# g1257/LanczosPlusPlus

Measured on AMD Instinct MI355X. Metric: Lanczos iterations/sec + SpMV achieved HBM GB/s vs roofline, 1/2/4/8 GPU, higher is better.
Workload: dtype f64

## Files before the change

lanczosplusplus_amd/csrc/lpp_pb_kernels.h:

```cpp
#pragma once
#include "lpp_kernels.h"
#include "lpp_pb_geom.h"

namespace lpp {

struct PbUpArgs {
	const uint32_t* tw;
	const int32_t* tw_off;
	const uint16_t* tw_len;
	int G;
	double gval[kPbMaxGroups];
	const double* dict;
	const uint8_t* dcode;
	int64_t n_up, pitch, n_blk;
	int spb;
	const double* y;
	double* u;
	double* partial;
	EpiScale sc;
	double* wbuf;
	double* ybuf;
	const double* g_a;
	const double* g_b2;
};

constexpr int kPbPreMax = 6;
constexpr int kPbPreMin = 1;
template <int GT> struct PbWords {
	uint2 w[GT][kPbPreMax];
	int nc[GT];
	double yo;
};

__device__ __forceinline__ uint32_t pb_lo8(uint32_t w)
{
	uint32_t r;
	asm("v_lshlrev_b32_sdwa %0, %1, %2 dst_sel:DWORD dst_unused:UNUSED_PAD src0_sel:DWORD src1_sel:WORD_0" : "=v"(r) : "v"(3u), "v"(w));
	return r;
}
__device__ __forceinline__ uint32_t pb_hi8(uint32_t w)
{
	uint32_t r;
	asm("v_lshlrev_b32_sdwa %0, %1, %2 dst_sel:DWORD dst_unused:UNUSED_PAD src0_sel:DWORD src1_sel:WORD_1" : "=v"(r) : "v"(3u), "v"(w));
	return r;
}
typedef __attribute__((address_space(3))) const double pb_lds_cdouble;
__device__ __forceinline__ double pb_lds_abs(uint32_t byte_addr) { return *(pb_lds_cdouble*)(uintptr_t)byte_addr; }

__device__ __forceinline__ void pb_lds_barrier()
{
	asm volatile("s_waitcnt lgkmcnt(0)" ::: "memory");
	__builtin_amdgcn_s_barrier();
}

template <bool DOT, int GT, bool CHAIN = false, int PRE0 = kPbPre> __global__ __launch_bounds__(kPbUpThreads, 4) void k_pb_up(PbUpArgs a)
{
	extern __shared__ __attribute__((aligned(16))) unsigned char lds_raw[];
	double* win = (double*)lds_raw;
	uint8_t* dcode_s = (uint8_t*)(win + a.pitch + kPbZeroSlots);
	int32_t* off_s = (int32_t*)(lds_raw + pb_up_meta_offset(a.pitch));
	uint16_t* len_s = (uint16_t*)(off_s + a.spb * a.G);
	double* dict_s = (double*)(lds_raw + pb_up_dict_offset(a.pitch, a.spb, a.G));
	double* smem = dict_s + 256;
	for (int i = threadIdx.x; i < 256; i += kPbUpThreads) dict_s[i] = a.dict[i];
	for (int i = threadIdx.x; i < a.spb * a.G; i += kPbUpThreads) {
		off_s[i] = a.tw_off[i];
		len_s[i] = a.tw_len[i];
	}
	double alpha, beta;
	epi_coeffs(a.sc, alpha, beta);
	double gco = 0.0;
	if (CHAIN && a.g_a) {
		gco = *a.g_a;
		const double b2 = *a.g_b2;
		if (sqrt(b2) >= 1e-10) gco /= b2;
	}
	constexpr int NW = kPbUpThreads / 64;
	constexpr int GG = GT > 0 ? GT : 1;
	const int lane = threadIdx.x & 63, wave = __builtin_amdgcn_readfirstlane((int)(threadIdx.x >> 6));
	const int p2 = (int)(a.pitch >> 1), p16 = (int)(a.pitch >> 4);
	double dot = 0.0;
	const uint2* const tw2 = (const uint2*)a.tw;
	const uint4* const tw4 = (const uint4*)a.tw;
	double* const uout = a.u;
	const int spb = a.spb, n_up = (int)a.n_up, G = a.G;
	double gv[GG];
#pragma unroll
	for (int g = 0; g < GG; g++) gv[g] = a.gval[g];
	auto gather4 = [=](const uint2& w, double& s0, double& s1) __attribute__((always_inline)) {
		s0 += pb_lds_abs(pb_lo8(w.x));
		s1 += pb_lds_abs(pb_hi8(w.x));
		s0 += pb_lds_abs(pb_lo8(w.y));
		s1 += pb_lds_abs(pb_hi8(w.y));
	};
	for (int64_t blk = blockIdx.x; blk < a.n_blk; blk += gridDim.x) {
		const double2* yb = (const double2*)(a.y + blk * a.pitch);
		const uint4* db = (const uint4*)(a.dcode + blk * a.pitch);
		const int64_t rowbase = blk * a.pitch;
		pb_lds_barrier();
		if (CHAIN) {
			double2* const wb = (double2*)(a.wbuf + rowbase);
			const double2* const yo = (const double2*)(a.ybuf + rowbase);
			const int di = min((int)threadIdx.x, p16 - 1);
			const uint4 dc0 = db[di];
			constexpr int NS = 4;
			for (int i0 = threadIdx.x; i0 < p2; i0 += NS * kPbUpThreads) {
				double2 wv[NS], yv[NS];
				int idx[NS];
#pragma unroll
				for (int q = 0; q < NS; q++) idx[q] = min(i0 + q * kPbUpThreads, p2 - 1);
#pragma unroll
				for (int q = 0; q < NS; q++) wv[q] = wb[idx[q]];
				if (gco != 0.0) {
#pragma unroll
					for (int q = 0; q < NS; q++) yv[q] = yo[idx[q]];
#pragma unroll
					for (int q = 0; q < NS; q++) {
						wv[q].x -= gco * yv[q].x;
						wv[q].y -= gco * yv[q].y;
						if (i0 + q * kPbUpThreads < p2) wb[idx[q]] = wv[q];
					}
				}
#pragma unroll
				for (int q = 0; q < NS; q++)
					if (i0 + q * kPbUpThreads < p2) ((double2*)win)[idx[q]] = wv[q];
			}
			((uint4*)dcode_s)[di] = dc0;
			for (int i0 = threadIdx.x + kPbUpThreads; i0 < p16; i0 += kPbUpThreads) ((uint4*)dcode_s)[i0] = db[i0];
		} else {
			constexpr int NS = 8;
			for (int pass = 0; pass < 8 / NS; pass++) {
				double2 t[NS];
				int idx[NS];
#pragma unroll
				for (int q = 0; q < NS; q++) idx[q] = min((int)threadIdx.x + (pass * NS + q) * kPbUpThreads, p2 - 1);
#pragma unroll
				for (int q = 0; q < NS; q++) t[q] = yb[idx[q]];
#pragma unroll
				for (int q = 0; q < NS; q++) ((double2*)win)[idx[q]] = t[q];
			}
			const int di = min((int)threadIdx.x, p16 - 1);
			((uint4*)dcode_s)[di] = db[di];
			for (int i0 = threadIdx.x + 8 * kPbUpThreads; i0 < p2; i0 += kPbUpThreads) ((double2*)win)[i0] = yb[i0];
			for (int i0 = threadIdx.x + kPbUpThreads; i0 < p16; i0 += kPbUpThreads) ((uint4*)dcode_s)[i0] = db[i0];
		}
		if (threadIdx.x < kPbZeroSlots) win[a.pitch + threadIdx.x] = 0.0;
		pb_lds_barrier();
		const double* const yold = CHAIN ? a.ybuf + rowbase : nullptr;
		auto own = [=](int j, double& yc, double& dv) __attribute__((always_inline)) {
			const int iu = min(j * 64 + lane, n_up - 1);
			yc = win[iu];
			dv = dict_s[dcode_s[iu]];
		};
		auto finish = [=, &dot](int j, double acc, double yc, double dv, double yo) __attribute__((always_inline)) {
			const int iu = j * 64 + lane;
			acc = fma(dv, yc, acc);
			if (iu < n_up) {
				const double uv = CHAIN ? fma(beta, yo, alpha * acc) : alpha * acc;
				__builtin_nontemporal_store(uv, &uout[rowbase + iu]);
				if (DOT) dot += yc * uv;
			}
		};
		auto epilogue = [=](int j, double acc, double yo = 0.0) __attribute__((always_inline)) {
			double yc, dv;
			own(j, yc, dv);
			finish(j, acc, yc, dv, yo);
		};
		if (GT > 0) {
			auto load_words = [=](int j, PbWords<GG>& s) __attribute__((always_inline)) {
#pragma unroll
				for (int g = 0; g < GG; g++) {
					s.nc[g] = __builtin_amdgcn_readfirstlane((int)len_s[j * GG + g]);
					constexpr int PRE0_ = PRE0;
					const int depth = pb_depth(GG, g, PRE0_);
					if (kPbPairs) {
						const uint4* wp4 = tw4 + (size_t)__builtin_amdgcn_readfirstlane(off_s[j * GG + g]) * 64 + lane;
#pragma unroll
						for (int c = 0; c < kPbPreMax; c += 2)
							if (c < depth) {
								const uint4 t = wp4[(c >> 1) * 64];
								s.w[g][c] = uint2 { t.x, t.y };
								s.w[g][c + 1] = uint2 { t.z, t.w };
							}
					} else {
						const uint2* wp = tw2 + (size_t)off_s[j * GG + g] * 64 + lane;
#pragma unroll
						for (int c = 0; c < kPbPreMax; c++)
							if (c < depth && (c < kPbPreMin || c < s.nc[g])) s.w[g][c] = wp[c * 64];
					}
				}
				if (CHAIN) s.yo = yold[min(j * 64 + lane, n_up - 1)];
			};
			auto group_sum = [=](int j, int g, int nc, const uint2* w, int depth) __attribute__((always_inline)) {
				double s0 = 0.0, s1 = 0.0;
				constexpr int BT = 2;
#pragma unroll
				for (int c = 0; c < kPbPreMax; c += BT) {
					if (c >= depth) continue;
					if (BT >= 3 && c + 3 <= depth && nc >= c + 3) {
						gather4(w[c], s0, s1);
						gather4(w[c + 1], s0, s1);
						gather4(w[c + 2], s0, s1);
					} else if (c + 2 <= depth && nc >= c + 2) {
						gather4(w[c], s0, s1);
						gather4(w[c + 1], s0, s1);
					} else if (nc >= c + 1) {
						gather4(w[c], s0, s1);
					}
				}
				if (nc > depth) {
					if (kPbPairs) {
						const uint4* wp4 = tw4 + (size_t)off_s[j * GG + g] * 64 + lane;
						for (int c = depth; c < nc; c += 2) {
							const uint4 t = wp4[(c >> 1) * 64];
							gather4(uint2 { t.x, t.y }, s0, s1);
							if (c + 1 < nc) gather4(uint2 { t.z, t.w }, s0, s1);
						}
					} else {
						const uint2* wp = tw2 + (size_t)off_s[j * GG + g] * 64 + lane;
						for (int c = depth; c < nc; c++) {
							const uint2 wr = wp[c * 64];
							gather4(wr, s0, s1);
						}
					}
				}
				return s0 + s1;
			};
			auto compute = [=](int j, const PbWords<GG>& s) __attribute__((always_inline)) {
				double yc, dv;
				own(j, yc, dv);
				double acc = 0.0;
#pragma unroll
				for (int g = 0; g < GG; g++) acc = fma(gv[g], group_sum(j, g, s.nc[g], s.w[g], pb_depth(GG, g, PRE0)), acc);
				if (kPbPairs) {
#pragma unroll
					for (int g = 0; g < GG; g++)
#pragma unroll
						for (int c = 0; c < kPbPreMax; c += 2)
							if (c < pb_depth(GG, g, PRE0)) asm volatile("" ::"v"(s.w[g][c].x));
				}
				if (CHAIN) asm volatile("" ::"v"(s.yo));
				finish(j, acc, yc, dv, CHAIN ? s.yo : 0.0);
			};
			PbWords<GG> wa, wb;
			int j = wave;
			if (j < spb) {
				load_words(j, wa);
				for (; j + 2 * NW < spb; j += 2 * NW) {
					load_words(j + NW, wb);
					compute(j, wa);
					load_words(j + 2 * NW, wa);
					compute(j + NW, wb);
				}
				if (j + NW < spb) {
					load_words(j + NW, wb);
					compute(j, wa);
					compute(j + NW, wb);
				} else {
					compute(j, wa);
				}
			}
		} else {
			for (int j = wave; j < spb; j += NW) {
				double acc = 0.0;
				const double yo_g = CHAIN ? yold[min(j * 64 + lane, n_up - 1)] : 0.0;
				uint2 wn[4];
				int ncn = __builtin_amdgcn_readfirstlane((int)len_s[j * G]);
				auto load4 = [=](size_t off, int c0, int nc, uint2* w) __attribute__((always_inline)) {
					if (kPbPairs) {
						const uint4* wp4 = tw4 + off * 64 + lane;
#pragma unroll
						for (int q = 0; q < 4; q += 2) {
							const uint4 t = wp4[((c0 + q) >> 1) * 64];
							w[q] = uint2 { t.x, t.y };
							w[q + 1] = uint2 { t.z, t.w };
						}
					} else {
						const uint2* wp = tw2 + off * 64 + lane;
#pragma unroll
						for (int q = 0; q < 4; q++)
							if (c0 + q < nc) w[q] = wp[(c0 + q) * 64];
					}
				};
				size_t offn = (size_t)__builtin_amdgcn_readfirstlane(off_s[j * G]);
				load4(offn, 0, ncn, wn);
				for (int g = 0; g < G; g++) {
					const int nc = ncn;
					const size_t off = offn;
					uint2 w[4];
#pragma unroll
					for (int q = 0; q < 4; q++) w[q] = wn[q];
					if (g + 1 < G) {
						ncn = __builtin_amdgcn_readfirstlane((int)len_s[j * G + g + 1]);
						offn = (size_t)__builtin_amdgcn_readfirstlane(off_s[j * G + g + 1]);
						load4(offn, 0, ncn, wn);
					}
					double s0 = 0.0, s1 = 0.0;
#pragma unroll
					for (int q = 0; q < 4; q++)
						if (q < nc) gather4(w[q], s0, s1);
					for (int c0 = 4; c0 < nc; c0 += 4) {
						uint2 wr[4];
						load4(off, c0, nc, wr);
#pragma unroll
						for (int q = 0; q < 4; q++)
							if (c0 + q < nc) gather4(wr[q], s0, s1);
						if (kPbPairs) asm volatile("" ::"v"(wr[0].x), "v"(wr[2].x));
					}
					acc = fma(a.gval[g], s0 + s1, acc);
				}
				epilogue(j, acc, yo_g);
			}
		}
	}
	if (DOT) {
		const double r = block_sum_n<kPbUpThreads / 64>(dot, smem);
		if (threadIdx.x == 0) a.partial[blockIdx.x] = r;
	}
}

template <int CTRL> __device__ __forceinline__ double dpp_shr(double v)
{
	const long long b = __double_as_longlong(v);
	const int lo = __builtin_amdgcn_update_dpp(0, (int)b, CTRL, 0xf, 0xf, true);
	const int hi = __builtin_amdgcn_update_dpp(0, (int)(b >> 32), CTRL, 0xf, 0xf, true);
	return __longlong_as_double((long long)(((unsigned long long)(unsigned)hi << 32) | (unsigned)lo));
}
__device__ __forceinline__ double wave_sum_rows(double v)
{
	v += dpp_shr<0x111>(v);
	v += dpp_shr<0x112>(v);
	v += dpp_shr<0x114>(v);
	v += dpp_shr<0x118>(v);
	auto lane_val = [&](int l) __attribute__((always_inline)) {
		const long long b = __double_as_longlong(v);
		const int lo = __builtin_amdgcn_readlane((int)b, l), hi = __builtin_amdgcn_readlane((int)(b >> 32), l);
		return __longlong_as_double((long long)(((unsigned long long)(unsigned)hi << 32) | (unsigned)lo));
	};
	return ((lane_val(15) + lane_val(31)) + lane_val(47)) + lane_val(63);
}

__device__ inline void pb_down_fill_image(uint32_t* row, int32_t* len, uint32_t* place, int stride, int rowcap, const int32_t* order, const int64_t* c_ptr,
                                          const int32_t* c_col, const uint8_t* c_code, int64_t b0, int nown, uint32_t rowmul, int tid, int nthreads)
{
	constexpr int BPT = 8;
	for (int il = tid; il < nown; il += nthreads) {
		const int64_t b = order[b0 + il];
		row[il] = (uint32_t)b * rowmul;
		len[il] = (int32_t)(c_ptr[b + 1] - c_ptr[b]);
	}
	for (int i = tid; i < nown * rowcap; i += nthreads) {
		const int il = i / rowcap, k = i - il * rowcap;
		const int64_t b = order[b0 + il];
		const int64_t p0 = c_ptr[b];
		const bool in = k < (int)(c_ptr[b + 1] - p0);
		const int64_t bl = order[b0 + (il & ~(BPT - 1))];
		const int64_t pl = c_ptr[bl];
		const int32_t fill = k < (int)(c_ptr[bl + 1] - pl) ? c_col[pl + k] : (int32_t)bl;
		place[il * stride + k] = ((uint32_t)(in ? c_col[p0 + k] : fill) & 0xffffffu) | ((uint32_t)(in ? c_code[p0 + k] : (uint8_t)0) << 24);
	}
}

struct PbDownArgs {
	int64_t pitch, n_blk;
	int npanels;
	int ids_per_wg;
	int rounds, ids_per_round;
	const uint4* image;
	int rowcap;
	const int64_t* c_ptr;
	const int32_t* c_col;
	const uint8_t* c_code;
	const int32_t* order;
	const double* dict;
	const double* y;
	double* z;
	const double* u_in;
	const double* shift;
	double* partial;
	EpiScale sc;
	int* pace;
	int u_has_beta;
	const double2* cdict;
	int pf_lead;
};

template <int THREADS, bool RMW = false, bool WIDE = false, bool CPLX = false, bool PF = false> __global__ __launch_bounds__(THREADS) void k_pb_down(PbDownArgs a)
{
	extern __shared__ __attribute__((aligned(16))) unsigned char lds_raw[];
	__shared__ double dict_s[CPLX ? 512 : 256];
	const int stride = pb_down_stride(a.rowcap);
	uint32_t* row_s = (uint32_t*)lds_raw;
	int32_t* len_s = (int32_t*)(row_s + a.ids_per_round);
	uint32_t* place_s = (uint32_t*)(lds_raw + (((size_t)a.ids_per_round * 8 + 15) & ~(size_t)15));
	__shared__ double smem_d[THREADS / 64];
	__shared__ int task_s[3];
	if (PF && threadIdx.x < 3) task_s[threadIdx.x] = 0;
	for (int i = threadIdx.x; i < (CPLX ? 512 : 256); i += THREADS) dict_s[i] = CPLX ? ((const double*)a.cdict)[i] : a.dict[i];
	double alpha, beta;
	epi_coeffs(a.sc, alpha, beta);
	double dot = 0.0, nrm = 0.0;
	const double sh = RMW ? *a.shift : 0.0;
	constexpr int LPL = 8;
	constexpr int BPT = 64 / LPL;
	constexpr int LSH = 7;
	const int lane = threadIdx.x & 63, wave = threadIdx.x >> 6, sub = lane / LPL, c = lane & (LPL - 1);
	const int nx = (gridDim.x & 7) == 0 ? 8 : 1;
	const int grp = nx == 8 ? (int)(blockIdx.x & 7) : 0;
	const int slot = nx == 8 ? (int)(blockIdx.x >> 3) : (int)blockIdx.x;
	const int nslots = (int)(gridDim.x / nx);
	const uint32_t rowbytes = WIDE ? (uint32_t)((a.pitch * 8) >> LSH) : (uint32_t)(a.pitch * 8);
	const int64_t b0w = (int64_t)slot * a.ids_per_wg;
	const int nown_w = (int)max((int64_t)0, min((int64_t)a.ids_per_wg, a.n_blk - b0w));
	const int rounds = a.rounds;
	const int tcap = (a.ids_per_round + BPT - 1) / BPT;
	double* const tsum_s = (double*)(lds_raw + pb_down_lds_bytes(a.ids_per_round, a.rowcap));
	auto fold = [&](int q, int ng) __attribute__((always_inline)) {
		if (wave != 0) return;
		const double* const t = tsum_s + (size_t)(q & 1) * 2 * tcap;
		double sd = 0.0, sn = 0.0;
		for (int i = lane; i < ng; i += 64) {
			sd += t[i];
			if (RMW) sn += t[tcap + i];
		}
		sd = wave_sum(sd);
		if (RMW) sn = wave_sum(sn);
		if (lane == 0) {
			dot += sd;
			nrm += sn;
		}
	};
	int64_t b0 = b0w;
	int nown = rounds == 1 ? nown_w : 0;
	auto build_image = [&](int r) __attribute__((always_inline)) {
		b0 = b0w + (int64_t)r * a.ids_per_round;
		nown = rounds == 1 ? nown_w : max(0, min(a.ids_per_round, nown_w - r * a.ids_per_round));
		if (rounds > 1 && a.image) {
			const int n4 = (int)(pb_down_lds_bytes(a.ids_per_round, a.rowcap) >> 4);
			const uint4* const src = a.image + ((size_t)slot * rounds + r) * (size_t)n4;
			for (int i = threadIdx.x; i < n4; i += THREADS) {
				uint4 v = src[i];
				if (4 * i < a.ids_per_round) {
					v.x *= rowbytes;
					v.y *= rowbytes;
					v.z *= rowbytes;
					v.w *= rowbytes;
				}
				((uint4*)lds_raw)[i] = v;
			}
			return;
		}
		pb_down_fill_image(row_s, len_s, place_s, stride, a.rowcap, a.order, a.c_ptr, a.c_col, a.c_code, b0, nown, rowbytes, (int)threadIdx.x, THREADS);
	};
	if (rounds == 1) build_image(0);
	__syncthreads();
	const char* ysrc = (const char*)a.y;
	for (int p = grp; p < a.npanels; p += nx) {
		if (a.pace && p >= grp + 2 * nx) {
			if (threadIdx.x == 0) {
				const int* cnt = a.pace + (int64_t)grp * a.npanels + (p - 2 * nx);
				for (int spin = 0; spin < 8192 && __hip_atomic_load(cnt, __ATOMIC_RELAXED, __HIP_MEMORY_SCOPE_AGENT) < nslots; spin++)
					__builtin_amdgcn_s_sleep(8);
			}
			__syncthreads();
		}
		const uint32_t colb = WIDE ? (uint32_t)(c * 16) : (uint32_t)((p << LSH) + c * 16);
		auto at = [=](uint32_t r) __attribute__((always_inline)) -> size_t { return WIDE ? (((size_t)(r + (uint32_t)p) << LSH) + colb) : (size_t)(r + colb); };
		const int pk = (p - grp) / nx;
		constexpr int NP = 8;
		uint32_t pft[PF ? NP : 1];
		if (PF && RMW) {
			if (wave == THREADS / 64 - 1 && nown > 0) {
				const bool nextp = p + nx < a.npanels;
#pragma unroll
				for (int k = 0; k < NP; k++) {
					const uint32_t r = row_s[min(lane + 64 * k, nown - 1)];
					const uint32_t pp = (uint32_t)(k < a.pf_lead && nextp ? p + nx : p);
					pft[k] = *(const uint32_t*)((const char*)a.u_in + (WIDE ? (((size_t)(r + pp)) << LSH) : (size_t)(r + (pp << LSH))));
				}
			}
		}
		for (int r = 0; r < rounds; r++) {
		if (rounds > 1) {
			__syncthreads();
			if (PF && r > 0) fold(pk * rounds + r - 1, (nown + BPT - 1) / BPT);
			build_image(r);
			__syncthreads();
		}
		const int ngroups = (nown + BPT - 1) / BPT;
		const int q = pk * rounds + r;
		if (PF && threadIdx.x == 0) task_s[(q + 2) % 3] = 0;
		auto next_task = [&](int prev) __attribute__((always_inline)) -> int {
			if (!PF) return prev < 0 ? wave : prev + THREADS / 64;
			int g = 0;
			if (lane == 0) g = atomicAdd(&task_s[q % 3], 1);
			return __builtin_amdgcn_readfirstlane(g);
		};
		for (int g = next_task(-1); g < ngroups; g = next_task(g)) {
			const int il = min(g * BPT + sub, nown - 1);
			const bool valid = g * BPT + sub < nown;
			const int n4 = (__builtin_amdgcn_readfirstlane(len_s[g * BPT]) + 3) >> 2;
			const uint4* const prow = (const uint4*)(place_s + il * stride);
			double2 acc = double2 { 0.0, 0.0 };
			double2 ga[4], gb[4], gc[4];
			uint4 pa, pb, pc;
			auto issue = [&](int ch, double2* gbuf, uint4& pw) __attribute__((always_inline)) {
				pw = prow[ch];
				const uint32_t w4[4] = { pw.x, pw.y, pw.z, pw.w };
#pragma unroll
				for (int q = 0; q < 4; q++) {
					gbuf[q] = *(const double2*)(ysrc + at((w4[q] & 0xffffffu) * rowbytes));
				}
			};
			auto consume = [&](const double2* gbuf, const uint4& pw) __attribute__((always_inline)) {
				const uint32_t w4[4] = { pw.x, pw.y, pw.z, pw.w };
#pragma unroll
				for (int q = 0; q < 4; q++) {
					if (CPLX) {
						const double2 v = ((const double2*)dict_s)[w4[q] >> 24];
						acc.x = fma(v.x, gbuf[q].x, fma(-v.y, gbuf[q].y, acc.x));
						acc.y = fma(v.x, gbuf[q].y, fma(v.y, gbuf[q].x, acc.y));
					} else {
						const double v = dict_s[w4[q] >> 24];
						acc.x = fma(v, gbuf[q].x, acc.x);
						acc.y = fma(v, gbuf[q].y, acc.y);
					}
				}
			};
			double2* const zp = (double2*)((char*)a.z + at(row_s[il]));
			double2 uo = double2 { 0.0, 0.0 }, xo = double2 { 0.0, 0.0 };
			if (RMW) {
				uo = nt_load2((const double2*)((const char*)a.u_in + at(row_s[il])));
				if (!a.u_has_beta) xo = nt_load2(zp);
			}
			if (n4 > 0) issue(0, ga, pa);
			if (n4 > 1) issue(1, gb, pb);
			for (int ch = 0; ch < n4; ch += 3) {
				if (ch + 2 < n4) issue(ch + 2, gc, pc);
				consume(ga, pa);
				if (ch + 1 < n4) {
					if (ch + 3 < n4) issue(ch + 3, ga, pa);
					consume(gb, pb);
				}
				if (ch + 2 < n4) {
					if (ch + 4 < n4) issue(ch + 4, gb, pb);
					consume(gc, pc);
				}
			}
			const double2 yown = *(const double2*)(ysrc + at(row_s[il]));
			double td = 0.0, tn = 0.0;
			if (valid) {
				acc.x = fma(alpha, acc.x, fma(beta, xo.x, uo.x));
				acc.y = fma(alpha, acc.y, fma(beta, xo.y, uo.y));
				__builtin_nontemporal_store(acc.x, &zp->x);
				__builtin_nontemporal_store(acc.y, &zp->y);
				td = yown.x * acc.x + yown.y * acc.y;
				if (RMW) {
					const double dx = acc.x - sh * yown.x, dy = acc.y - sh * yown.y;
					tn = dx * dx + dy * dy;
				}
			}
			if (PF) {
				double* const t = tsum_s + (size_t)(q & 1) * 2 * tcap;
				td = wave_sum_rows(td);
				if (RMW) tn = wave_sum_rows(tn);
				if (lane == 0) {
					t[g] = td;
					if (RMW) t[tcap + g] = tn;
				}
			} else {
				dot += td;
				nrm += tn;
			}
		}
		}
		if (PF && RMW && wave == THREADS / 64 - 1 && nown > 0) {
			uint32_t x = 0;
#pragma unroll
			for (int k = 0; k < NP; k++) x ^= pft[k];
			asm volatile("" ::"v"(x));
		}
		if (a.pace || PF) {
			__syncthreads();
			if (a.pace && threadIdx.x == 0) __hip_atomic_fetch_add(a.pace + (int64_t)grp * a.npanels + p, 1, __ATOMIC_RELAXED, __HIP_MEMORY_SCOPE_AGENT);
			if (PF) fold(pk * rounds + rounds - 1, (nown + BPT - 1) / BPT);
		}
	}
	if (a.partial) {
		const double r = block_sum_n<THREADS / 64>(dot, smem_d);
		if (threadIdx.x == 0) a.partial[RMW ? 2 * blockIdx.x : blockIdx.x] = r;
		if (RMW) {
			const double q = block_sum_n<THREADS / 64>(nrm, smem_d);
			if (threadIdx.x == 0) a.partial[2 * blockIdx.x + 1] = q;
		}
	}
}

static __global__ __launch_bounds__(256) void k_pb_down_image(PbDownArgs a, uint4* out)
{
	const int slot = (int)blockIdx.x / a.rounds, r = (int)blockIdx.x - slot * a.rounds;
	const int64_t b0w = (int64_t)slot * a.ids_per_wg;
	const int nown_w = (int)max((int64_t)0, min((int64_t)a.ids_per_wg, a.n_blk - b0w));
	const int nown = max(0, min(a.ids_per_round, nown_w - r * a.ids_per_round));
	const size_t bytes = pb_down_lds_bytes(a.ids_per_round, a.rowcap);
	unsigned char* const img = (unsigned char*)out + (size_t)blockIdx.x * bytes;
	uint32_t* const row = (uint32_t*)img;
	int32_t* const len = (int32_t*)(row + a.ids_per_round);
	uint32_t* const place = (uint32_t*)(img + (((size_t)a.ids_per_round * 8 + 15) & ~(size_t)15));
	pb_down_fill_image(row, len, place, pb_down_stride(a.rowcap), a.rowcap, a.order, a.c_ptr, a.c_col, a.c_code, b0w + (int64_t)r * a.ids_per_round, nown, 1u, (int)threadIdx.x, 256);
}

static __global__ __launch_bounds__(kBlock) void k_pb_materialise(double2* __restrict__ y, const double2* __restrict__ x, const double* __restrict__ g_a,
                                                                  const double* __restrict__ g_b2, int64_t n2, double* __restrict__ partial)
{
	__shared__ double smem[kBlock / 64];
	double g = *g_a;
	const double b2 = *g_b2;
	if (sqrt(b2) >= 1e-10) g /= b2;
	double c = 0.0;
	for (int64_t i = (int64_t)blockIdx.x * kBlock + threadIdx.x; i < n2; i += (int64_t)gridDim.x * kBlock) {
		const double2 xv = x[i];
		double2 yv = y[i];
		yv.x -= g * xv.x;
		yv.y -= g * xv.y;
		y[i] = yv;
		c += yv.x * xv.x + yv.y * xv.y;
	}
	const double r = block_sum(c, smem);
	if (threadIdx.x == 0) partial[blockIdx.x] = r;
}

struct PbCombineArgs {
	double2* x;
	const double2 *y, *u, *z;
	const double2* d;
	double* partial_dq;
	int64_t n2;
	EpiScale sc;
	const double* a_ptr;
	const double* b2_prev;
	double* partial_nrm;
	double* partial_xy;
};

static __global__ __launch_bounds__(kBlock) void k_pb_combine(PbCombineArgs a)
{
	__shared__ double smem[kBlock / 64];
	double alpha, beta;
	epi_coeffs(a.sc, alpha, beta);
	const bool hasd = a.d != nullptr;
	const bool hasz = a.z != nullptr;
	double g = 0.0;
	if (a.a_ptr) {
		g = *a.a_ptr;
		if (a.b2_prev) {
			const double b2 = *a.b2_prev;
			if (sqrt(b2) >= 1e-10) g /= b2;
		}
	}
	double s = 0.0, c = 0.0, q = 0.0;
	const int64_t stride = (int64_t)gridDim.x * kBlock;
	int64_t i = (int64_t)blockIdx.x * kBlock + threadIdx.x;
	constexpr int U = 4;
	for (; i + (U - 1) * stride < a.n2; i += U * stride) {
		double2 xv[U], yv[U], uv[U], zv[U];
#pragma unroll
		for (int k = 0; k < U; k++) xv[k] = nt_load2(&a.x[i + k * stride]);
#pragma unroll
		for (int k = 0; k < U; k++) yv[k] = nt_load2(&a.y[i + k * stride]);
#pragma unroll
		for (int k = 0; k < U; k++) uv[k] = nt_load2(&a.u[i + k * stride]);
#pragma unroll
		for (int k = 0; k < U; k++) zv[k] = hasz ? nt_load2(&a.z[i + k * stride]) : double2 { 0.0, 0.0 };
		double2 dv[U];
		if (hasd) {
#pragma unroll
			for (int k = 0; k < U; k++) dv[k] = nt_load2(&a.d[i + k * stride]);
		}
#pragma unroll
		for (int k = 0; k < U; k++) {
			double2 r;
			r.x = beta * xv[k].x + uv[k].x + zv[k].x - g * yv[k].x;
			r.y = beta * xv[k].y + uv[k].y + zv[k].y - g * yv[k].y;
			if (hasd) {
				r.x = fma(alpha * dv[k].x, yv[k].x, r.x);
				r.y = fma(alpha * dv[k].y, yv[k].y, r.y);
				q += dv[k].x * r.x * r.x + dv[k].y * r.y * r.y;
			}
			nt_store2(r, &a.x[i + k * stride]);
			s += r.x * r.x + r.y * r.y;
			c += r.x * yv[k].x + r.y * yv[k].y;
		}
	}
	for (; i < a.n2; i += stride) {
		const double2 xv = a.x[i], yv = a.y[i], uv = a.u[i], zv = hasz ? a.z[i] : double2 { 0.0, 0.0 };
		double2 r;
		r.x = beta * xv.x + uv.x + zv.x - g * yv.x;
		r.y = beta * xv.y + uv.y + zv.y - g * yv.y;
		if (hasd) {
			const double2 dv = a.d[i];
			r.x = fma(alpha * dv.x, yv.x, r.x);
			r.y = fma(alpha * dv.y, yv.y, r.y);
			q += dv.x * r.x * r.x + dv.y * r.y * r.y;
		}
		a.x[i] = r;
		s += r.x * r.x + r.y * r.y;
		c += r.x * yv.x + r.y * yv.y;
	}
	if (a.partial_nrm) {
		const double rs = block_sum(s, smem);
		if (threadIdx.x == 0) a.partial_nrm[blockIdx.x] = rs;
		const double rc = block_sum(c, smem);
		if (threadIdx.x == 0) a.partial_xy[blockIdx.x] = rc;
	}
	if (a.partial_dq) {
		const double rq = block_sum(q, smem);
		if (threadIdx.x == 0) a.partial_dq[blockIdx.x] = rq;
	}
}

static __global__ __launch_bounds__(kBlock) void k_pb_unpack_combine(double2* __restrict__ x, const double2* __restrict__ y, const double2* __restrict__ u,
                                                                     const double2* __restrict__ recv, int64_t nblk, int64_t pitch2, int64_t peru2, int64_t chunk2,
                                                                     EpiScale sc, double* __restrict__ partial, const double* __restrict__ shift,
                                                                     const double2* __restrict__ dplain = nullptr)
{
	__shared__ double smem[kBlock / 64];
	double alpha, beta;
	epi_coeffs(sc, alpha, beta);
	const double sh = shift ? *shift : 0.0;
	const int64_t n2 = nblk * pitch2;
	double dot = 0.0, nrm = 0.0;
	for (int64_t i = (int64_t)blockIdx.x * kBlock + threadIdx.x; i < n2; i += (int64_t)gridDim.x * kBlock) {
		const int64_t b = i / pitch2, c = i - b * pitch2;
		const int64_t p = c / peru2, cl = c - p * peru2;
		const double2 zv = recv[p * chunk2 + b * peru2 + cl];
		const double2 xv = x[i], uv = u[i], yv = y[i];
		double2 r;
		r.x = beta * xv.x + uv.x + zv.x;
		r.y = beta * xv.y + uv.y + zv.y;
		if (dplain) {
			const double2 dv = dplain[i];
			r.x = fma(alpha * dv.x, yv.x, r.x);
			r.y = fma(alpha * dv.y, yv.y, r.y);
		}
		x[i] = r;
		dot += yv.x * r.x + yv.y * r.y;
		const double dx = r.x - sh * yv.x, dy = r.y - sh * yv.y;
		nrm += dx * dx + dy * dy;
	}
	const double rd = block_sum(dot, smem);
	if (threadIdx.x == 0) partial[2 * blockIdx.x] = rd;
	const double rn = block_sum(nrm, smem);
	if (threadIdx.x == 0) partial[2 * blockIdx.x + 1] = rn;
}

static __global__ __launch_bounds__(kBlock) void k_pb_dq(const double2* __restrict__ y, const double2* __restrict__ d, int64_t n2, double* __restrict__ partial)
{
	__shared__ double smem[kBlock / 64];
	double q = 0.0;
	for (int64_t i = (int64_t)blockIdx.x * kBlock + threadIdx.x; i < n2; i += (int64_t)gridDim.x * kBlock) {
		const double2 yv = y[i], dv = d[i];
		q += dv.x * yv.x * yv.x + dv.y * yv.y * yv.y;
	}
	const double r = block_sum(q, smem);
	if (threadIdx.x == 0) partial[blockIdx.x] = r;
}

static __global__ __launch_bounds__(kBlock) void k_pb_reduce_a(const double* __restrict__ partial, int np, const double* __restrict__ xy, EpiScale sc,
                                                               double* __restrict__ out)
{
	__shared__ double smem[kBlock / 64];
	double alpha, beta;
	epi_coeffs(sc, alpha, beta);
	double s = 0.0;
	for (int p = threadIdx.x; p < np; p += kBlock) s += partial[p];
	const double r = block_sum(s, smem);
	if (threadIdx.x == 0) out[0] = r + beta * xy[0] + alpha * xy[1];
}


static __global__ void k_pb_rebuild(int64_t n_up, int64_t n_blk, int64_t pitch, const int64_t* __restrict__ t_ptr, const int32_t* __restrict__ t_col,
                                    const double* __restrict__ t_val, const int64_t* __restrict__ c_ptr, const int32_t* __restrict__ c_col,
                                    const uint8_t* __restrict__ c_code, const int64_t* __restrict__ blockbase, const uint8_t* __restrict__ dcode,
                                    const double* __restrict__ dict, int64_t* __restrict__ rowptr_out, int32_t* __restrict__ col_out,
                                    double* __restrict__ val_out, const double* __restrict__ dplain = nullptr, const int32_t* __restrict__ inv = nullptr)
{
	const int64_t r = (int64_t)blockIdx.x * blockDim.x + threadIdx.x;
	const int64_t n = n_up * n_blk;
	if (r == 0 && rowptr_out) rowptr_out[n] = blockbase[n_blk];
	if (r >= n) return;
	const int64_t b = r / n_up, i = r - b * n_up;
	const int64_t c0 = c_ptr[b], c1 = c_ptr[b + 1];
	int64_t o = blockbase[b] + t_ptr[i] + i * (1 + (c1 - c0));
	if (rowptr_out) rowptr_out[r] = o;
	if (!col_out) return;
	int64_t p = c0;
	for (; p < c1 && c_col[p] < b; p++, o++) {
		col_out[o] = (int32_t)((int64_t)c_col[p] * n_up + i);
		val_out[o] = dict[c_code[p]];
	}
	int64_t q = t_ptr[i];
	const int64_t q1 = t_ptr[i + 1];
	for (; q < q1 && t_col[q] < i; q++, o++) {
		col_out[o] = (int32_t)(b * n_up + t_col[q]);
		val_out[o] = t_val[q];
	}
	col_out[o] = (int32_t)r;
	const int64_t at = b * pitch + (inv ? inv[i] : i);
	val_out[o] = dplain ? dplain[at] : dict[dcode[at]];
	o++;
	for (; q < q1; q++, o++) {
		col_out[o] = (int32_t)(b * n_up + t_col[q]);
		val_out[o] = t_val[q];
	}
	for (; p < c1; p++, o++) {
		col_out[o] = (int32_t)((int64_t)c_col[p] * n_up + i);
		val_out[o] = dict[c_code[p]];
	}
}


static __global__ void k_pb_rebuild_c(int64_t n_up, int64_t n_blk, int64_t pitch, const int64_t* __restrict__ t_ptr, const int32_t* __restrict__ t_col,
                                    const double2* __restrict__ t_val, const int64_t* __restrict__ c_ptr, const int32_t* __restrict__ c_col,
                                    const uint8_t* __restrict__ c_code, const int64_t* __restrict__ blockbase, const uint8_t* __restrict__ dcode,
                                    const double* __restrict__ dict, const double2* __restrict__ cdict, int64_t* __restrict__ rowptr_out, int32_t* __restrict__ col_out,
                                    double2* __restrict__ val_out, const double* __restrict__ dplain = nullptr, const int32_t* __restrict__ inv = nullptr)
{
	const int64_t r = (int64_t)blockIdx.x * blockDim.x + threadIdx.x;
	const int64_t n = n_up * n_blk;
	if (r == 0 && rowptr_out) rowptr_out[n] = blockbase[n_blk];
	if (r >= n) return;
	const int64_t b = r / n_up, i = r - b * n_up;
	const int64_t c0 = c_ptr[b], c1 = c_ptr[b + 1];
	int64_t o = blockbase[b] + t_ptr[i] + i * (1 + (c1 - c0));
	if (rowptr_out) rowptr_out[r] = o;
	if (!col_out) return;
	int64_t p = c0;
	for (; p < c1 && c_col[p] < b; p++, o++) {
		col_out[o] = (int32_t)((int64_t)c_col[p] * n_up + i);
		val_out[o] = cdict[c_code[p]];
	}
	int64_t q = t_ptr[i];
	const int64_t q1 = t_ptr[i + 1];
	for (; q < q1 && t_col[q] < i; q++, o++) {
		col_out[o] = (int32_t)(b * n_up + t_col[q]);
		val_out[o] = t_val[q];
	}
	col_out[o] = (int32_t)r;
	const int64_t at = b * pitch + 2 * i;
	val_out[o] = double2 { dplain ? dplain[at] : dict[dcode[at]], 0.0 };
	o++;
	for (; q < q1; q++, o++) {
		col_out[o] = (int32_t)(b * n_up + t_col[q]);
		val_out[o] = t_val[q];
	}
	for (; p < c1; p++, o++) {
		col_out[o] = (int32_t)((int64_t)c_col[p] * n_up + i);
		val_out[o] = cdict[c_code[p]];
	}
}



template <bool FILL, typename V = double>
static __global__ void k_pb_csr_couplings(int64_t n_up, int64_t n_blk, const int64_t* __restrict__ rowptr, const int32_t* __restrict__ col,
                                          const V* __restrict__ val, int64_t* __restrict__ c_len, const int64_t* __restrict__ c_ptr,
                                          int32_t* __restrict__ c_col, V* __restrict__ c_val, int* __restrict__ bad)
{
	const int64_t b = (int64_t)blockIdx.x * blockDim.x + threadIdx.x;
	if (b >= n_blk) return;
	const int64_t r = b * n_up;
	int64_t n = 0;
	for (int64_t p = rowptr[r]; p < rowptr[r + 1]; p++) {
		const int64_t c = col[p];
		if (c >= r && c < r + n_up) continue;
		if (c % n_up != 0) *bad = 1;
		if (FILL) {
			c_col[c_ptr[b] + n] = (int32_t)(c / n_up);
			c_val[c_ptr[b] + n] = val[p];
		}
		n++;
	}
	if (!FILL) c_len[b] = n;
}

static __global__ void k_pb_csr_diagonal(int64_t n_up, int64_t n_blk, int64_t pitch, const int64_t* __restrict__ rowptr, const int32_t* __restrict__ col,
                                         const double* __restrict__ val, double* __restrict__ dval, int* __restrict__ bad)
{
	const int64_t n = n_up * n_blk;
	for (int64_t r = (int64_t)blockIdx.x * blockDim.x + threadIdx.x; r < n; r += (int64_t)gridDim.x * blockDim.x) {
		bool found = false;
		for (int64_t p = rowptr[r]; p < rowptr[r + 1]; p++)
			if ((int64_t)col[p] == r) {
				dval[(r / n_up) * pitch + (r % n_up)] = val[p];
				found = true;
				break;
			}
		if (!found) *bad = 1;
	}
}

static __global__ void k_pb_csr_diagonal_c(int64_t n_c, int64_t n_blk, int64_t pitch, const int64_t* __restrict__ rowptr, const int32_t* __restrict__ col,
                                           const double2* __restrict__ val, double* __restrict__ dval, int* __restrict__ bad)
{
	const int64_t n = n_c * n_blk;
	for (int64_t r = (int64_t)blockIdx.x * blockDim.x + threadIdx.x; r < n; r += (int64_t)gridDim.x * blockDim.x) {
		bool found = false;
		for (int64_t p = rowptr[r]; p < rowptr[r + 1]; p++)
			if ((int64_t)col[p] == r) {
				const double2 v = val[p];
				if (__double_as_longlong(v.y) != 0) *bad = 1;
				const int64_t at = (r / n_c) * pitch + 2 * (r % n_c);
				dval[at] = v.x;
				dval[at + 1] = v.x;
				found = true;
				break;
			}
		if (!found) *bad = 1;
	}
}

static __global__ void k_pb_codes_from_values(int64_t n, const double* __restrict__ dval, const double* __restrict__ dict, int ndict, uint8_t* __restrict__ dcode)
{
	for (int64_t k = (int64_t)blockIdx.x * blockDim.x + threadIdx.x; k < n; k += (int64_t)gridDim.x * blockDim.x) dcode[k] = (uint8_t)dict_code(dict, ndict, dval[k]);
}

static __global__ void k_pb_csr_verify(int64_t n_up, int64_t n_blk, int64_t pitch, const int64_t* __restrict__ t_ptr, const int32_t* __restrict__ t_col,
                                       const double* __restrict__ t_val, const int64_t* __restrict__ c_ptr, const int32_t* __restrict__ c_col,
                                       const uint8_t* __restrict__ c_code, const int64_t* __restrict__ blockbase, const uint8_t* __restrict__ dcode,
                                       const double* __restrict__ dict, const double* __restrict__ dplain, const int64_t* __restrict__ rowptr,
                                       const int32_t* __restrict__ col, const double* __restrict__ val, int* __restrict__ bad,
                                       const int32_t* __restrict__ inv = nullptr)
{
	const int64_t n = n_up * n_blk;
	for (int64_t r = (int64_t)blockIdx.x * blockDim.x + threadIdx.x; r < n; r += (int64_t)gridDim.x * blockDim.x) {
		const int64_t b = r / n_up, i = r - b * n_up;
		const int64_t dat = b * pitch + (inv ? inv[i] : i);
		const int64_t c0 = c_ptr[b], c1 = c_ptr[b + 1];
		int64_t o = blockbase[b] + t_ptr[i] + i * (1 + (c1 - c0));
		const int64_t oe = o + (t_ptr[i + 1] - t_ptr[i]) + 1 + (c1 - c0);
		bool ok = rowptr[r] == o && rowptr[r + 1] == oe;
		if (ok) {
			auto same = [&](int64_t at, int64_t c, double v) { return (int64_t)col[at] == c && __double_as_longlong(val[at]) == __double_as_longlong(v); };
			int64_t p = c0;
			for (; p < c1 && c_col[p] < b; p++, o++) ok = ok && same(o, (int64_t)c_col[p] * n_up + i, dict[c_code[p]]);
			int64_t q = t_ptr[i];
			const int64_t q1 = t_ptr[i + 1];
			for (; q < q1 && t_col[q] < i; q++, o++) ok = ok && same(o, b * n_up + t_col[q], t_val[q]);
			ok = ok && same(o, r, dplain ? dplain[dat] : dict[dcode[dat]]);
			o++;
			for (; q < q1; q++, o++) ok = ok && same(o, b * n_up + t_col[q], t_val[q]);
			for (; p < c1; p++, o++) ok = ok && same(o, (int64_t)c_col[p] * n_up + i, dict[c_code[p]]);
		}
		if (!ok) *bad = 1;
	}
}

static __global__ void k_pb_csr_verify_c(int64_t n_up, int64_t n_blk, int64_t pitch, const int64_t* __restrict__ t_ptr, const int32_t* __restrict__ t_col,
                                       const double2* __restrict__ t_val, const int64_t* __restrict__ c_ptr, const int32_t* __restrict__ c_col,
                                       const uint8_t* __restrict__ c_code, const int64_t* __restrict__ blockbase, const uint8_t* __restrict__ dcode,
                                       const double* __restrict__ dict, const double2* __restrict__ cdict, const double* __restrict__ dplain, const int64_t* __restrict__ rowptr,
                                       const int32_t* __restrict__ col, const double2* __restrict__ val, int* __restrict__ bad)
{
	const int64_t n = n_up * n_blk;
	for (int64_t r = (int64_t)blockIdx.x * blockDim.x + threadIdx.x; r < n; r += (int64_t)gridDim.x * blockDim.x) {
		const int64_t b = r / n_up, i = r - b * n_up;
		const int64_t dat = b * pitch + 2 * i;
		const int64_t c0 = c_ptr[b], c1 = c_ptr[b + 1];
		int64_t o = blockbase[b] + t_ptr[i] + i * (1 + (c1 - c0));
		const int64_t oe = o + (t_ptr[i + 1] - t_ptr[i]) + 1 + (c1 - c0);
		bool ok = rowptr[r] == o && rowptr[r + 1] == oe;
		if (ok) {
			auto same = [&](int64_t at, int64_t c, double2 v) { return (int64_t)col[at] == c && __double_as_longlong(val[at].x) == __double_as_longlong(v.x) && __double_as_longlong(val[at].y) == __double_as_longlong(v.y); };
			int64_t p = c0;
			for (; p < c1 && c_col[p] < b; p++, o++) ok = ok && same(o, (int64_t)c_col[p] * n_up + i, cdict[c_code[p]]);
			int64_t q = t_ptr[i];
			const int64_t q1 = t_ptr[i + 1];
			for (; q < q1 && t_col[q] < i; q++, o++) ok = ok && same(o, b * n_up + t_col[q], t_val[q]);
			ok = ok && same(o, r, double2 { dplain ? dplain[dat] : dict[dcode[dat]], 0.0 });
			o++;
			for (; q < q1; q++, o++) ok = ok && same(o, b * n_up + t_col[q], t_val[q]);
			for (; p < c1; p++, o++) ok = ok && same(o, (int64_t)c_col[p] * n_up + i, cdict[c_code[p]]);
		}
		if (!ok) *bad = 1;
	}
}

template <bool TO_STORED>
static __global__ void k_pb_permute(double* __restrict__ dst, const double* __restrict__ src, const int32_t* __restrict__ perm, int64_t n_blk, int64_t rows,
                                    int64_t pitch)
{
	const int64_t n = n_blk * pitch;
	for (int64_t k = (int64_t)blockIdx.x * blockDim.x + threadIdx.x; k < n; k += (int64_t)gridDim.x * blockDim.x) {
		const int64_t b = k / pitch, p = k - b * pitch;
		if (p >= rows) {
			dst[k] = 0.0;
			continue;
		}
		if (TO_STORED) dst[k] = src[b * pitch + perm[p]];
		else dst[b * pitch + perm[p]] = src[k];
	}
}

static __global__ void k_fill_random_pitched(double* __restrict__ v, int64_t n_blk, int64_t rows, int64_t pitch, int64_t offset, uint64_t seed,
                                             const int32_t* __restrict__ perm = nullptr)
{
	const int64_t n = n_blk * pitch;
	for (int64_t k = (int64_t)blockIdx.x * blockDim.x + threadIdx.x; k < n; k += (int64_t)gridDim.x * blockDim.x) {
		const int64_t b = k / pitch, i = k - b * pitch;
		double val = 0.0;
		if (i < rows) {
			const uint64_t r = splitmix64(seed * 0x2545F4914F6CDD1DULL + (uint64_t)(b * rows + (perm ? perm[i] : i) + offset));
			val = (double)(r >> 11) * (1.0 / 9007199254740992.0) - 0.5;
		}
		v[k] = val;
	}
}

}
```

Before: 362.5.

## Prefetch next block's old vector and codes, stage wbuf via global_load_lds

In the CHAIN path of the up-kernel, the next grid-stride block's ybuf slice and first dcode words are now requested into registers during the tail of the current block's compute, hiding their latency behind the gather work. The wbuf window is staged directly into LDS with global_load_lds, and the gco*yold subtraction is applied in place in LDS and written back. This adds register pressure (NS double2 values held across the compute loop), a full vmcnt(0) wait per staging chunk, and more complex control flow around idle waves.

Measured after the change: 367.9, median of 6. 1.01x the previous value.

```diff
diff --git a/lanczosplusplus_amd/csrc/lpp_pb_kernels.h b/lanczosplusplus_amd/csrc/lpp_pb_kernels.h
--- a/lanczosplusplus_amd/csrc/lpp_pb_kernels.h
+++ b/lanczosplusplus_amd/csrc/lpp_pb_kernels.h
@@ -53,6 +53,12 @@
 	__builtin_amdgcn_s_barrier();
 }
 
+__device__ __forceinline__ void pb_wait_vm0()
+{
+	__builtin_amdgcn_s_waitcnt(0x0F70);
+	asm volatile("" ::: "memory");
+}
+
 template <bool DOT, int GT, bool CHAIN = false, int PRE0 = kPbPre> __global__ __launch_bounds__(kPbUpThreads, 4) void k_pb_up(PbUpArgs a)
 {
 	extern __shared__ __attribute__((aligned(16))) unsigned char lds_raw[];
@@ -93,6 +99,25 @@
 		s0 += pb_lds_abs(pb_lo8(w.y));
 		s1 += pb_lds_abs(pb_hi8(w.y));
 	};
+	constexpr int NS = GT == 2 && PRE0 >= 6 ? 6 : 7;
+	double2 yv[NS] = {};
+	uint4 dc0 = {};
+	const bool sub = gco != 0.0;
+	const double* const ybuf = a.ybuf;
+	const uint8_t* const dcode_g = a.dcode;
+	const int64_t pitch = a.pitch, n_blk = a.n_blk;
+	auto request_old = [=](int64_t nb, double2(&yq)[NS], uint4& dc) __attribute__((always_inline)) {
+		const bool live = nb < n_blk;
+		const int64_t base = (live ? nb : n_blk - 1) * pitch;
+		const int my = live && sub ? -1 : 0, md = live ? -1 : 0;
+		int t = threadIdx.x;
+		asm volatile("" : "+v"(t));
+		dc = ((const uint4*)(dcode_g + base))[min(t, p16 - 1) & md];
+		const double2* const yo = (const double2*)(ybuf + base);
+#pragma unroll
+		for (int q = 0; q < NS; q++) yq[q] = yo[min(t + q * kPbUpThreads, p2 - 1) & my];
+	};
+	if (CHAIN) request_old(blockIdx.x, yv, dc0);
 	for (int64_t blk = blockIdx.x; blk < a.n_blk; blk += gridDim.x) {
 		const double2* yb = (const double2*)(a.y + blk * a.pitch);
 		const uint4* db = (const uint4*)(a.dcode + blk * a.pitch);
@@ -100,32 +125,40 @@
 		pb_lds_barrier();
 		if (CHAIN) {
 			double2* const wb = (double2*)(a.wbuf + rowbase);
-			const double2* const yo = (const double2*)(a.ybuf + rowbase);
-			const int di = min((int)threadIdx.x, p16 - 1);
-			const uint4 dc0 = db[di];
-			constexpr int NS = 4;
-			for (int i0 = threadIdx.x; i0 < p2; i0 += NS * kPbUpThreads) {
-				double2 wv[NS], yv[NS];
-				int idx[NS];
-#pragma unroll
-				for (int q = 0; q < NS; q++) idx[q] = min(i0 + q * kPbUpThreads, p2 - 1);
-#pragma unroll
-				for (int q = 0; q < NS; q++) wv[q] = wb[idx[q]];
-				if (gco != 0.0) {
-#pragma unroll
-					for (int q = 0; q < NS; q++) yv[q] = yo[idx[q]];
+			double2* const win2 = (double2*)win;
+			auto stage_row = [=](int i0, int ldsbase, const double2(&yq)[NS]) __attribute__((always_inline)) {
+#pragma unroll
+				for (int q = 0; q < NS; q++)
+					if (i0 + q * kPbUpThreads < p2)
+						__builtin_amdgcn_global_load_lds(wb + i0 + q * kPbUpThreads, (__attribute__((address_space(3))) void*)(uintptr_t)(uint32_t)((ldsbase + q * kPbUpThreads) * 16), 16, 0, 0);
+				pb_wait_vm0();
+				if (sub) {
 #pragma unroll
 					for (int q = 0; q < NS; q++) {
-						wv[q].x -= gco * yv[q].x;
-						wv[q].y -= gco * yv[q].y;
-						if (i0 + q * kPbUpThreads < p2) wb[idx[q]] = wv[q];
+						const int i = i0 + q * kPbUpThreads;
+						if (i < p2) {
+							double2 wv = win2[i];
+							wv.x -= gco * yq[q].x;
+							wv.y -= gco * yq[q].y;
+							win2[i] = wv;
+							wb[i] = wv;
+						}
 					}
 				}
-#pragma unroll
-				for (int q = 0; q < NS; q++)
-					if (i0 + q * kPbUpThreads < p2) ((double2*)win)[idx[q]] = wv[q];
-			}
-			((uint4*)dcode_s)[di] = dc0;
+			};
+			int t0 = threadIdx.x;
+			asm volatile("" : "+v"(t0));
+			stage_row(t0, wave * 64, yv);
+			((uint4*)dcode_s)[min(t0, p16 - 1)] = dc0;
+			for (int i0 = threadIdx.x + NS * kPbUpThreads; i0 < p2; i0 += NS * kPbUpThreads) {
+				const double2* const yo = (const double2*)(ybuf + rowbase);
+				double2 yt[NS] = {};
+				if (sub) {
+#pragma unroll
+					for (int q = 0; q < NS; q++) yt[q] = yo[min(i0 + q * kPbUpThreads, p2 - 1)];
+				}
+				stage_row(i0, __builtin_amdgcn_readfirstlane(i0 - lane), yt);
+			}
 			for (int i0 = threadIdx.x + kPbUpThreads; i0 < p16; i0 += kPbUpThreads) ((uint4*)dcode_s)[i0] = db[i0];
 		} else {
 			constexpr int NS = 8;
@@ -252,13 +285,24 @@
 					load_words(j + 2 * NW, wa);
 					compute(j + NW, wb);
 				}
-				if (j + NW < spb) {
+				if (CHAIN) {
+					const bool two = j + NW < spb;
+					load_words(two ? j + NW : j, wb);
+					request_old(blk + gridDim.x, yv, dc0);
+					compute(j, wa);
+					if (two) compute(j + NW, wb);
+				} else if (j + NW < spb) {
 					load_words(j + NW, wb);
 					compute(j, wa);
 					compute(j + NW, wb);
 				} else {
 					compute(j, wa);
 				}
+			}
+			if (CHAIN) {
+				int idle = __builtin_amdgcn_readfirstlane((int)(wave >= spb));
+				asm volatile("" : "+s"(idle));
+				if (idle) request_old(blk + gridDim.x, yv, dc0);
 			}
 		} else {
 			for (int j = wave; j < spb; j += NW) {
@@ -311,6 +355,7 @@
 				}
 				epilogue(j, acc, yo_g);
 			}
+			if (CHAIN) request_old(blk + gridDim.x, yv, dc0);
 		}
 	}
 	if (DOT) {
```
